# yoxu515/aot-benchmark

Hardware: NVIDIA H100
Metric: frames/sec (480p, 10 obj) (higher is better)
Workload: dtype f32

## Files before the change

### aot_benchmark_b200/csrc/conv_tc.cu

```cuda
#include <type_traits>

#include "common.cuh"
#include "tc_common.cuh"

namespace aotb {
namespace tc {

constexpr int CONV_A_BYTES = 128 * 128;

template <int BN>
__device__ __forceinline__ void wgmma_conv(float* acc, uint64_t a, uint64_t b) {
    if (BN == 256) wgmma_ss_n256(acc, a, b, 1u);
    else if (BN == 128) wgmma_ss_n128(acc, a, b, 1u);
    else wgmma_ss_n64(acc, a, b, 1u);
}

template <int BN>
__device__ __forceinline__ void conv_acc_to_staging(const float* acc, float* stg, int ld) {
    const int warp = threadIdx.x >> 5, lane = threadIdx.x & 31;
    const int row0 = (warp >> 2) * 64 + (warp & 3) * 16 + (lane >> 2), cq = (lane & 3) * 2;
#pragma unroll
    for (int j = 0; j < BN / 2; j += 2)
        *reinterpret_cast<float2*>(stg + (row0 + 8 * ((j >> 1) & 1)) * ld + 8 * (j >> 2) + cq) = make_float2(acc[j], acc[j + 1]);
}

struct ConvTcArgs {
    const float* in;
    const float* bias;
    const float* wscale;
    const float* res;
    float* out;
    int B, H, W, Cin, ldin;
    int Ho, Wo, Cout, ldout, ldres;
    int KH, KW, stride, pad;
    int M, nchunks;
    int act;
    int splits;
    int spin;
    long long* prof;
};

static int g_conv_tiling = 0;

struct RowInfo { int pix_base, iy0, ix0, valid; };

template <int BN, int S, int NB>
__device__ __forceinline__ void conv_finish_tile(const ConvTcArgs& a, const uint8_t* smem, int tid, int m0, int n0, int zrank) {
    constexpr int LD = BN + 4, C4 = BN / 4, RSTEP = 256 / C4, ROWS = 128 / S, ITERS = ROWS / RSTEP;
    constexpr int B = NB < ITERS ? NB : ITERS;
    static_assert(ITERS >= 1 && ITERS % B == 0, "finish tiling");
    const int c = (tid % C4) * 4, n = n0 + c;
    const int r0 = zrank * ROWS + tid / C4;
    const float4 b4 = a.bias ? __ldg(reinterpret_cast<const float4*>(a.bias + n)) : make_float4(0.f, 0.f, 0.f, 0.f);
    const float4 s4 = a.wscale ? __ldg(reinterpret_cast<const float4*>(a.wscale + n)) : make_float4(1.f, 1.f, 1.f, 1.f);
    const float* lbase = reinterpret_cast<const float*>(smem) + r0 * LD + c;
    const uint32_t sbase = smem_u32(lbase);
#pragma unroll 1
    for (int i0 = 0; i0 < ITERS; i0 += B) {
        float4 v[B][S], rs[B];
#pragma unroll
        for (int b = 0; b < B; ++b) {
            const int ro = (i0 + b) * RSTEP;
            if (S == 1) {
                v[b][0] = *reinterpret_cast<const float4*>(lbase + ro * LD);
            } else {
#pragma unroll
                for (int z = 0; z < S; ++z) v[b][z] = dsmem_ld_f4(dsmem_addr(sbase + (uint32_t)(ro * LD) * 4u, (uint32_t)z));
            }
            const int m = m0 + r0 + ro;
            rs[b] = (a.res && m < a.M) ? *reinterpret_cast<const float4*>(a.res + (size_t)m * a.ldres + n)
                                       : make_float4(0.f, 0.f, 0.f, 0.f);
        }
#pragma unroll
        for (int b = 0; b < B; ++b) {
            float4 o = v[b][0];
#pragma unroll
            for (int z = 1; z < S; ++z) { o.x += v[b][z].x; o.y += v[b][z].y; o.z += v[b][z].z; o.w += v[b][z].w; }
            o.x = fmaf(o.x, s4.x, b4.x); o.y = fmaf(o.y, s4.y, b4.y); o.z = fmaf(o.z, s4.z, b4.z); o.w = fmaf(o.w, s4.w, b4.w);
            o.x += rs[b].x; o.y += rs[b].y; o.z += rs[b].z; o.w += rs[b].w;
            o.x = apply_act(o.x, a.act); o.y = apply_act(o.y, a.act);
            o.z = apply_act(o.z, a.act); o.w = apply_act(o.w, a.act);
            const int m = m0 + r0 + (i0 + b) * RSTEP;
            if (m < a.M) *reinterpret_cast<float4*>(a.out + (size_t)m * a.ldout + n) = o;
        }
    }
}

template <int BN>
struct FinishPre { static constexpr int B = BN == 256 ? 4 : 8; float4 b4, s4; float4 rs[B]; };

template <int BN>
__device__ __forceinline__ void finish_prefetch(const ConvTcArgs& a, int tid, int m0, int n0, FinishPre<BN>& pre) {
    constexpr int C4 = BN / 4, RSTEP = 256 / C4;
    const int n = n0 + (tid % C4) * 4, r0 = tid / C4;
    pre.b4 = a.bias ? __ldg(reinterpret_cast<const float4*>(a.bias + n)) : make_float4(0.f, 0.f, 0.f, 0.f);
    pre.s4 = a.wscale ? __ldg(reinterpret_cast<const float4*>(a.wscale + n)) : make_float4(1.f, 1.f, 1.f, 1.f);
#pragma unroll
    for (int b = 0; b < FinishPre<BN>::B; ++b) {
        const int m = m0 + r0 + b * RSTEP;
        pre.rs[b] = (a.res && m < a.M) ? *reinterpret_cast<const float4*>(a.res + (size_t)m * a.ldres + n)
                                       : make_float4(0.f, 0.f, 0.f, 0.f);
    }
}

template <int BN>
__device__ __forceinline__ void conv_finish_tile_pre(const ConvTcArgs& a, const uint8_t* smem, int tid, int m0, int n0,
                                                     const FinishPre<BN>& pre) {
    constexpr int LD = BN + 4, C4 = BN / 4, RSTEP = 256 / C4, ITERS = 128 / RSTEP, B = FinishPre<BN>::B;
    static_assert(ITERS % B == 0, "finish tiling");
    const int c = (tid % C4) * 4, n = n0 + c, r0 = tid / C4;
    const uint32_t sbase = smem_u32(reinterpret_cast<const float*>(smem) + r0 * LD + c);
    float4 rs[B];
#pragma unroll
    for (int b = 0; b < B; ++b) rs[b] = pre.rs[b];
#pragma unroll 1
    for (int i0 = 0; i0 < ITERS; i0 += B) {
        float4 v[B], nx[B];
#pragma unroll
        for (int b = 0; b < B; ++b)
            asm volatile("ld.shared.v4.f32 {%0, %1, %2, %3}, [%4];" : "=f"(v[b].x), "=f"(v[b].y), "=f"(v[b].z), "=f"(v[b].w)
                         : "r"(sbase + (uint32_t)((i0 + b) * RSTEP * LD) * 4u));
        if (i0 + B < ITERS) {
#pragma unroll
            for (int b = 0; b < B; ++b) {
                const int m = m0 + r0 + (i0 + B + b) * RSTEP;
                nx[b] = (a.res && m < a.M) ? *reinterpret_cast<const float4*>(a.res + (size_t)m * a.ldres + n)
                                           : make_float4(0.f, 0.f, 0.f, 0.f);
            }
        }
#pragma unroll
        for (int b = 0; b < B; ++b) {
            float4 o = v[b];
            o.x = fmaf(o.x, pre.s4.x, pre.b4.x); o.y = fmaf(o.y, pre.s4.y, pre.b4.y);
            o.z = fmaf(o.z, pre.s4.z, pre.b4.z); o.w = fmaf(o.w, pre.s4.w, pre.b4.w);
            o.x += rs[b].x; o.y += rs[b].y; o.z += rs[b].z; o.w += rs[b].w;
            o.x = apply_act(o.x, a.act); o.y = apply_act(o.y, a.act);
            o.z = apply_act(o.z, a.act); o.w = apply_act(o.w, a.act);
            const int m = m0 + r0 + (i0 + b) * RSTEP;
            if (m < a.M) *reinterpret_cast<float4*>(a.out + (size_t)m * a.ldout + n) = o;
        }
        if (i0 + B < ITERS) {
#pragma unroll
            for (int b = 0; b < B; ++b) rs[b] = nx[b];
        }
    }
}

template <int BN, int STAGES, bool SPLIT>
struct ConvSmem {
    static constexpr int A_BYTES = CONV_A_BYTES;
    static constexpr int B_BYTES = BN * 128;
    static constexpr int PARTS = SPLIT ? 2 : 1;
    static constexpr int STAGE_BYTES = PARTS * A_BYTES + PARTS * B_BYTES;
    static constexpr int STG_LD = BN + 4;
    static_assert(128 * STG_LD * 4 <= STAGES * STAGE_BYTES, "staging tile must fit in the operand stages");
    static constexpr int TOTAL = STAGES * STAGE_BYTES + 128 * (int)sizeof(RowInfo) + 3 * STAGES * 8 + 1024;
    static_assert(TOTAL <= 227 * 1024, "shared memory of one CTA");
};

template <int BN, int STAGES, bool SPLIT>
__global__ void __launch_bounds__(384, 1)
conv_tc_kernel(const __grid_constant__ CUtensorMap tmWh, const __grid_constant__ CUtensorMap tmWl, const ConvTcArgs a) {
    using SM = ConvSmem<BN, STAGES, SPLIT>;
    extern __shared__ uint8_t smem_raw[];
    uint8_t* smem = reinterpret_cast<uint8_t*>((reinterpret_cast<uintptr_t>(smem_raw) + 1023) & ~(uintptr_t)1023);
    RowInfo* rinfo = reinterpret_cast<RowInfo*>(smem + STAGES * SM::STAGE_BYTES);
    uint64_t* a_full = reinterpret_cast<uint64_t*>(rinfo + 128);
    uint64_t* b_full = a_full + STAGES;
    uint64_t* s_free = b_full + STAGES;

    const int tid = threadIdx.x, warp = tid >> 5;
    const int m0 = blockIdx.x * 128, n0 = blockIdx.y * BN;
    long long* prof = a.prof ? a.prof + 12 * ((size_t)(blockIdx.z * gridDim.y + blockIdx.y) * gridDim.x + blockIdx.x) : nullptr;
    auto stamp = [&](int slot) { if (prof) prof[slot] = clock64(); };
    if (tid == 0) stamp(0);
    pdl_trigger();

    if (tid == 0) {
        for (int s = 0; s < STAGES; ++s) { mbar_init(&a_full[s], 128); mbar_init(&b_full[s], 1); mbar_init(&s_free[s], 8); }
        fence_mbar_init();
    }
    if (tid < 128) {
        const int m = m0 + tid;
        RowInfo ri;
        if (m < a.M) {
            const int HoWo = a.Ho * a.Wo;
            const int b = m / HoWo, r = m - b * HoWo;
            const int oy = r / a.Wo, ox = r - oy * a.Wo;
            ri.pix_base = b * a.H * a.W;
            ri.iy0 = oy * a.stride - a.pad;
            ri.ix0 = ox * a.stride - a.pad;
            ri.valid = 1;
        } else {
            ri.pix_base = 0; ri.iy0 = 0; ri.ix0 = 0; ri.valid = 0;
        }
        rinfo[tid] = ri;
    }
    __syncthreads();
    if (tid == 0) stamp(1);
    pdl_wait();
    const int cpt = (a.Cin % 64 == 0) ? (a.Cin >> 6) : 0;
    const int per = (a.nchunks + a.splits - 1) / a.splits;
    const int kbeg = blockIdx.z * per;
    const int nloc = max(0, min(per, a.nchunks - kbeg));

    FinishPre<BN> pre;
    const int wg = __shfl_sync(0xffffffffu, tid >> 7, 0);
    if (wg < 2) {
        const uint64_t dA0 = smem_desc_sw128(smem_u32(smem + wg * 64 * 128));
        const uint64_t dB0 = smem_desc_sw128(smem_u32(smem + SM::PARTS * SM::A_BYTES));
        float acc[BN / 2];
#pragma unroll
        for (int j = 0; j < BN / 2; ++j) acc[j] = 0.f;
#pragma unroll 1
        for (int it = 0; it < nloc; ++it) {
            const int s = it % STAGES;
            const uint32_t ph = (it / STAGES) & 1;
            mbar_wait_cp(&a_full[s], ph, a.spin);
            mbar_wait_cp(&b_full[s], ph, a.spin);
            if (it == 0 && tid == 0) stamp(3);
            const uint64_t so = (uint64_t)((s * SM::STAGE_BYTES) >> 4);
            const uint64_t ah = dA0 + so, al = ah + (SM::A_BYTES >> 4), bh = dB0 + so, bl = bh + (uint64_t)(SM::B_BYTES >> 4);
            reg_fence<BN / 2>(acc);
            wgmma_fence();
#pragma unroll
            for (int ks = 0; ks < 4; ++ks) {
                wgmma_conv<BN>(acc, ah + 2 * ks, bh + 2 * ks);
                if constexpr (SPLIT) {
                    wgmma_conv<BN>(acc, al + 2 * ks, bh + 2 * ks);
                    wgmma_conv<BN>(acc, ah + 2 * ks, bl + 2 * ks);
                }
            }
            wgmma_commit();
            reg_fence<BN / 2>(acc);
            wgmma_wait<1>();
            if (it > 0) mbar_arrive_warp(&s_free[(it - 1) % STAGES]);
        }
        wgmma_wait<0>();
        reg_fence<BN / 2>(acc);
        if (tid == 0) stamp(4);
        if (a.splits == 1) finish_prefetch<BN>(a, tid, m0, n0, pre);
        asm volatile("bar.sync 1, 256;" ::: "memory");
        conv_acc_to_staging<BN>(acc, reinterpret_cast<float*>(smem), SM::STG_LD);
        if (tid == 0) stamp(6);
    } else {
        const int p = tid - 256, q = p & 15, rsub = p >> 4;
        const uint32_t soff = rsub * 128 + (((q >> 1) ^ rsub) << 4) + ((q & 1) << 3);
        const float4* in4 = reinterpret_cast<const float4*>(a.in);
        uint32_t off[16];
        int cur_tap = -1, c4 = 0;
        if (p == 0) { tma_prefetch_desc(&tmWh); if constexpr (SPLIT) tma_prefetch_desc(&tmWl); }
        auto load_half = [&](int h, auto part_c, float4* v) {
            constexpr int part = decltype(part_c)::value;
            if (part == 0) {
                const int kc = kbeg + (h >> 1);
                int tap, c0;
                if (cpt > 0) { tap = kc / cpt; c0 = ((kc - tap * cpt) << 6) + q * 4; }
                else { const int k = kc * 64 + q * 4; tap = k / a.Cin; c0 = k - tap * a.Cin; }
                c4 = c0 >> 2;
                if (tap != cur_tap) {
                    cur_tap = tap;
                    const bool kvalid = tap < a.KH * a.KW;
                    const int ky = tap / a.KW, kx = tap - ky * a.KW;
#pragma unroll
                    for (int i = 0; i < 16; ++i) {
                        const RowInfo ri = rinfo[rsub + i * 8];
                        const int iy = ri.iy0 + ky, ix = ri.ix0 + kx;
                        off[i] = (kvalid && ri.valid && iy >= 0 && iy < a.H && ix >= 0 && ix < a.W)
                                     ? (uint32_t)(((size_t)(ri.pix_base + iy * a.W + ix) * a.ldin) >> 2)
                                     : ~0u;
                    }
                }
            }
#pragma unroll
            for (int i = 0; i < 8; ++i) {
                const uint32_t o = off[part * 8 + i];
                v[i] = o != ~0u ? __ldg(in4 + ((size_t)o + c4)) : make_float4(0.f, 0.f, 0.f, 0.f);
            }
        };
        auto store_half = [&](int h, auto part_c, const float4* v) {
            constexpr int part = decltype(part_c)::value;
            const int it = h >> 1, s = it % STAGES;
            uint8_t* stage = smem + s * SM::STAGE_BYTES;
            if (part == 0) {
                if (it >= STAGES) mbar_wait_cp(&s_free[s], ((it / STAGES) - 1) & 1, a.spin);
                if (p == 0) {
                    uint8_t* Bh = stage + SM::PARTS * SM::A_BYTES;
                    mbar_arrive_expect_tx(&b_full[s], SM::PARTS * SM::B_BYTES);
                    tma_load_2d(Bh, &tmWh, &b_full[s], (kbeg + it) * 64, n0);
                    if constexpr (SPLIT) tma_load_2d(Bh + SM::B_BYTES, &tmWl, &b_full[s], (kbeg + it) * 64, n0);
                }
            }
            uint8_t* Ah = stage + part * 64 * 128 + soff;
            uint8_t* Al = Ah + SM::A_BYTES;
#pragma unroll
            for (int i = 0; i < 8; ++i) {
                const __half2 h0 = __floats2half2_rn(v[i].x, v[i].y), h1 = __floats2half2_rn(v[i].z, v[i].w);
                if constexpr (!SPLIT) {
                    uint2 ph;
                    ph.x = *reinterpret_cast<const uint32_t*>(&h0); ph.y = *reinterpret_cast<const uint32_t*>(&h1);
                    *reinterpret_cast<uint2*>(Ah + i * 1024) = ph;
                    continue;
                }
                const __half2 l0 = __floats2half2_rn(v[i].x - __low2float(h0), v[i].y - __high2float(h0));
                const __half2 l1 = __floats2half2_rn(v[i].z - __low2float(h1), v[i].w - __high2float(h1));
                uint2 ph, pl;
                ph.x = *reinterpret_cast<const uint32_t*>(&h0); ph.y = *reinterpret_cast<const uint32_t*>(&h1);
                pl.x = *reinterpret_cast<const uint32_t*>(&l0); pl.y = *reinterpret_cast<const uint32_t*>(&l1);
                *reinterpret_cast<uint2*>(Ah + i * 1024) = ph;
                *reinterpret_cast<uint2*>(Al + i * 1024) = pl;
            }
            if (part == 1) {
                fence_proxy_async();
                mbar_arrive(&a_full[s]);
                if (it == 0 && p == 0) stamp(2);
            }
        };
        using P0 = std::integral_constant<int, 0>;
        using P1 = std::integral_constant<int, 1>;
        const int nh = 2 * nloc;
        float4 v0[8], v1[8], v2[8];
        if (nh > 0) { load_half(0, P0{}, v0); load_half(1, P1{}, v1); }
#pragma unroll 1
        for (int h = 0; h < nh; h += 6) {
            if (h + 2 < nh) load_half(h + 2, P0{}, v2);
            store_half(h, P0{}, v0);
            if (h + 3 < nh) load_half(h + 3, P1{}, v0);
            store_half(h + 1, P1{}, v1);
            if (h + 2 < nh) {
                if (h + 4 < nh) load_half(h + 4, P0{}, v1);
                store_half(h + 2, P0{}, v2);
                if (h + 5 < nh) load_half(h + 5, P1{}, v2);
                store_half(h + 3, P1{}, v0);
            }
            if (h + 4 < nh) {
                if (h + 6 < nh) load_half(h + 6, P0{}, v0);
                store_half(h + 4, P0{}, v1);
                if (h + 7 < nh) load_half(h + 7, P1{}, v1);
                store_half(h + 5, P1{}, v2);
            }
        }
        if (p == 0) stamp(5);
    }
    __syncwarp();
    if (a.splits > 1) cluster_sync_all(); else __syncthreads();
    if (tid == 0) stamp(8);
    if (warp < 8) {
        const int zr = a.splits > 1 ? (int)blockIdx.z : 0;
        if (a.splits == 1) conv_finish_tile_pre<BN>(a, smem, tid, m0, n0, pre);
        else if (a.splits == 2) conv_finish_tile<BN, 2, 4>(a, smem, tid, m0, n0, zr);
        else if (a.splits == 4) conv_finish_tile<BN, 4, 2>(a, smem, tid, m0, n0, zr);
        else conv_finish_tile<BN, 8, 2>(a, smem, tid, m0, n0, zr);
    }
    if (tid == 0) stamp(9);
    if (a.splits > 1) {
        __syncwarp();
        cluster_sync_all();
    }
    if (tid == 0) stamp(7);
}

static int make_tmap_weights(CUtensorMap* out, const void* base, int Kpad, int Cout, int BN) {
    PFN_encodeTiled fn = tensor_map_encoder();
    if (!fn) return AOTB_ERR_CUDA;
    cuuint64_t dims[2] = {(cuuint64_t)Kpad, (cuuint64_t)Cout};
    cuuint64_t strides[1] = {(cuuint64_t)Kpad * 2};
    cuuint32_t box[2] = {64, (cuuint32_t)BN};
    cuuint32_t estr[2] = {1, 1};
    CUresult r = fn(out, CU_TENSOR_MAP_DATA_TYPE_FLOAT16, 2, const_cast<void*>(base), dims, strides, box, estr,
                    CU_TENSOR_MAP_INTERLEAVE_NONE, CU_TENSOR_MAP_SWIZZLE_128B, CU_TENSOR_MAP_L2_PROMOTION_L2_256B,
                    CU_TENSOR_MAP_FLOAT_OOB_FILL_NONE);
    if (r != CUDA_SUCCESS) {
        set_error("cuTensorMapEncodeTiled(weights) failed (%d)", (int)r);
        return AOTB_ERR_CUDA;
    }
    return AOTB_OK;
}

template <int BN, int STAGES, bool SPLIT>
static int launch_conv_tc(const CUtensorMap& th, const CUtensorMap& tl, const ConvTcArgs& a, cudaStream_t st) {
    constexpr int smem = ConvSmem<BN, STAGES, SPLIT>::TOTAL;
    static bool configured = false;
    if (!configured) {
        cudaError_t e = cudaFuncSetAttribute(conv_tc_kernel<BN, STAGES, SPLIT>, cudaFuncAttributeMaxDynamicSharedMemorySize,
                                             smem);
        if (e != cudaSuccess) {
            set_error("aotb_conv2d_nhwc_tc: cudaFuncSetAttribute: %s", cudaGetErrorString(e));
            return AOTB_ERR_CUDA;
        }
        configured = true;
    }
    dim3 grid(cdiv(a.M, 128), a.Cout / BN, a.splits);
    launch_cluster(conv_tc_kernel<BN, STAGES, SPLIT>, dim3(grid), dim3(384), smem, st, a.splits, th, tl, a);
    return check_launch("aotb_conv2d_nhwc_tc");
}

}
}

using namespace aotb;

extern "C" int aotb_set_conv_tiling(int mode) {
    AOTB_REQUIRE(mode >= 0 && mode < (1 << 12), "aotb_set_conv_tiling: mode is a 12-bit mask");
    tc::g_conv_tiling = mode;
    return AOTB_OK;
}

extern "C" int aotb_conv2d_nhwc_tc(const float* in, const void* wh, const void* wl, const float* bias, const float* wscale,
                                   const float* res, float* out, int B, int H, int W, int Cin, int ldin, int Cout, int ldout, int ldres,
                                   int KH, int KW, int stride, int pad, int act, void* workspace, size_t workspace_bytes,
                                   void* stream) {
    AOTB_REQUIRE(in && wh && out, "aotb_conv2d_nhwc_tc: null pointer");
    const bool split = wl != nullptr;
    AOTB_REQUIRE(Cin % 4 == 0 && Cout % 64 == 0, "aotb_conv2d_nhwc_tc: Cin must be a multiple of 4, Cout of 64");
    AOTB_REQUIRE(act >= aotb::ACT_NONE && act <= aotb::ACT_RELU6, "aotb_conv2d_nhwc_tc: activation %d not supported (0-4)", act);
    AOTB_REQUIRE(ldin % 4 == 0 && ldout % 4 == 0 && (!res || ldres % 4 == 0) && ((uintptr_t)in % 16 == 0) &&
                     ((uintptr_t)out % 16 == 0) && (!res || (uintptr_t)res % 16 == 0) && (!bias || (uintptr_t)bias % 16 == 0) &&
                     (!wscale || (uintptr_t)wscale % 16 == 0),
                 "aotb_conv2d_nhwc_tc: 16-byte alignment required");
    AOTB_REQUIRE((size_t)B * H * W * ldin / 4 < 0xFFFFFFFFull, "aotb_conv2d_nhwc_tc: input larger than 2^32 float4");
    tc::ConvTcArgs a;
    a.in = in; a.bias = bias; a.wscale = wscale; a.res = res; a.out = out;
    a.B = B; a.H = H; a.W = W; a.Cin = Cin; a.ldin = ldin;
    a.Ho = (H + 2 * pad - KH) / stride + 1;
    a.Wo = (W + 2 * pad - KW) / stride + 1;
    AOTB_REQUIRE(a.Ho > 0 && a.Wo > 0, "aotb_conv2d_nhwc_tc: empty output");
    a.Cout = Cout; a.ldout = ldout; a.ldres = ldres; a.KH = KH; a.KW = KW; a.stride = stride; a.pad = pad;
    a.M = B * a.Ho * a.Wo;
    const int K = ((KH * KW * Cin + 63) / 64) * 64;
    a.nchunks = K / 64;
    a.act = act;
    const int mt = cdiv(a.M, 128);
    int BN = 64, best_s = 1;
    const float kGather = 2.5f, kGather1 = 2.0f;
    if ((tc::g_conv_tiling & 1) == 0) {
        float best = 1e30f;
        const int bns[3] = {256, 128, 64};
        const float t_chunk[3] = {fmaxf(kGather, 4.0f), fmaxf(kGather, 2.0f), fmaxf(kGather, 1.0f)};
        const float t_chunk1[3] = {fmaxf(kGather1, 4.0f / 3), fmaxf(kGather1, 2.0f / 3), fmaxf(kGather1, 1.0f / 3)};
        const float t_fin[3] = {8.0f, 4.0f, 2.0f};
        for (int bi = 0; bi < 3; ++bi) {
            if (Cout % bns[bi]) continue;
            for (int sp = 1; sp <= 8; sp <<= 1) {
                if (sp > a.nchunks) break;
                const int ctas = mt * (Cout / bns[bi]) * sp;
                const int slots = sp == 8 ? 128 : 132;
                if (sp > 1 && ctas > slots) continue;
                const int waves = cdiv(ctas, slots);
                const float t = waves * (3.0f + cdiv(a.nchunks, sp) * (split ? t_chunk[bi] : t_chunk1[bi]) + t_fin[bi]);
                if (t < best) { best = t; BN = bns[bi]; best_s = sp; }
            }
        }
    } else {
        if (Cout % 128 == 0 && mt * (Cout / 128) >= 120) BN = 128;
        const int ctas = mt * (Cout / BN);
        if (ctas < 100 && a.nchunks >= 4) {
            best_s = 8;
            while (best_s > 1 && (ctas * best_s > 160 || a.nchunks / best_s < 2)) best_s >>= 1;
        }
    }
    const int force_bn = (tc::g_conv_tiling >> 4) & 15, force_s = (tc::g_conv_tiling >> 8) & 15;
    if (force_bn) {
        BN = 32 << force_bn;
        AOTB_REQUIRE((BN == 64 || BN == 128 || BN == 256) && Cout % BN == 0, "aotb_conv2d_nhwc_tc: forced tile %d invalid", BN);
    }
    a.splits = force_bn ? 1 : best_s;
    const int ctas = mt * (Cout / BN);
    if (force_s) {
        AOTB_REQUIRE((force_s == 1 || force_s == 2 || force_s == 4 || force_s == 8) && force_s <= a.nchunks,
                     "aotb_conv2d_nhwc_tc: forced split %d invalid", force_s);
        a.splits = force_s;
    }
    a.spin = (tc::g_conv_tiling & 2) ? 1 : 0;
    a.prof = nullptr;
    if (tc::g_conv_tiling & 4) {
        const size_t need = (size_t)ctas * a.splits * 12 * sizeof(long long);
        AOTB_REQUIRE(workspace && workspace_bytes >= need, "aotb_conv2d_nhwc_tc: profile mode needs %zu workspace bytes", need);
        a.prof = (long long*)workspace;
    }
    CUtensorMap th, tl;
    int rc;
    if ((rc = tc::make_tmap_weights(&th, wh, K, Cout, BN)) != AOTB_OK) return rc;
    cudaStream_t st = (cudaStream_t)stream;
    if (!split) {
        if (BN == 256) return tc::launch_conv_tc<256, 4, false>(th, th, a, st);
        if (BN == 128) return tc::launch_conv_tc<128, 6, false>(th, th, a, st);
        return tc::launch_conv_tc<64, 8, false>(th, th, a, st);
    }
    if ((rc = tc::make_tmap_weights(&tl, wl, K, Cout, BN)) != AOTB_OK) return rc;
    if (BN == 256) return tc::launch_conv_tc<256, 2, true>(th, tl, a, st);
    if (BN == 128) return tc::launch_conv_tc<128, 3, true>(th, tl, a, st);
    return tc::launch_conv_tc<64, 4, true>(th, tl, a, st);
}
```

### aot_benchmark_b200/ops.py

```python
from __future__ import annotations

import contextlib
import os

import torch

from ._lib import AotbError, check, lib

ACT_NONE, ACT_RELU, ACT_GELU, ACT_SILU, ACT_RELU6, ACT_HSWISH = 0, 1, 2, 3, 4, 5
EW_COPY, EW_ADD, EW_MUL, EW_SILU, EW_SILU_MUL, EW_FILL = 0, 1, 2, 3, 4, 5


def _st(stream):
    return torch.cuda.current_stream().cuda_stream if stream is None else stream


def _chk(*ts):
    for t in ts:
        if t is None:
            continue
        if not t.is_cuda or t.dtype != torch.float32:
            raise AotbError(f"aot_benchmark_b200 kernels need float32 CUDA tensors, got {t.dtype} on {t.device}")
        if t.dim() >= 1 and t.stride(-1) != 1:
            raise AotbError("innermost stride must be 1")
# ... 67 lines not shown
        wt = torch.nn.functional.pad(wt, (0, 64 - K % 64))
    hi = wt.half()
    lo = (wt - hi.float()).half()
    return hi.contiguous(), lo.contiguous()


def weight_scale_exponents(w_kn):
    amax = w_kn.abs().amax(dim=0).float()
    _, ex = torch.frexp(amax)
    e = (14 - ex).clamp(max=126)
    return torch.where(amax > 0, e, torch.zeros_like(e)).to(torch.int32)


def split_fp16_scaled(w_kn):
    e = weight_scale_exponents(w_kn)
    hi, lo = split_fp16(w_kn.float() * _pow2(e))
    return hi, lo, _pow2(-e)


def _pow2(e):
    return ((e + 127) << 23).to(torch.int32).view(torch.float32)


CONV_CHAIN = False


def conv2d_tc(x, wh, wl, bias, out, res=None, KH=1, KW=1, stride=1, pad=0, act=ACT_NONE, stream=None, wscale=None):
    _chk(x, bias, out, res, wscale)
    B, H, W, Cin = x.shape
    Cout = wh.shape[0]
    ws = _tc_workspace(x.device)
    with _ConvProbe(2.0 * out.shape[0] * out.shape[1] * out.shape[2] * Cout * KH * KW * Cin, stream):
        check(lib().aotb_conv2d_nhwc_tc(_p(x), wh.data_ptr(), _p(wl), _p(bias), _p(wscale), _p(res), _p(out), B, H, W, Cin,
                                        _nhwc_ld(x), Cout, _nhwc_ld(out), _nhwc_ld(res) if res is not None else 0, KH, KW,
                                        stride, pad, act, ws.data_ptr(), ws.numel(), _st(stream)), "aotb_conv2d_nhwc_tc")
    return out


def conv2d(x, w, bias, out, res=None, KH=1, KW=1, stride=1, pad=0, dil=1, act=ACT_NONE, stream=None):
    if CONV_IMPL == "tc" and dil == 1:
        t = _TC_WEIGHTS.get(w.data_ptr())
        if t is not None:
            return conv2d_tc(x, t[0], None if _PRECISION == "fp16" else t[1], bias, out, res=res, KH=KH, KW=KW, stride=stride, pad=pad, act=act,
                             stream=stream, wscale=t[2])
    _chk(x, w, bias, out, res)
    B, H, W, Cin = x.shape
    Cout = w.shape[1]
    check(lib().aotb_conv2d_nhwc_f32(_p(x), _p(w), _p(bias), _p(res), _p(out), B, H, W, Cin, _nhwc_ld(x), Cout,
                                     _nhwc_ld(out), _nhwc_ld(res) if res is not None else 0, KH, KW, stride, pad,
                                     dil, act, _st(stream)), "aotb_conv2d_nhwc_f32")
    return out


def linear(x, wt, bias, out, res=None, act=ACT_NONE, stream=None):
    if CONV_IMPL == "tc":
        t = _TC_WEIGHTS.get(wt.data_ptr())
        if t is not None:
            _chk(x, bias, out, res, t[2])
            M, K = x.shape
            N = wt.shape[1]
            ws = _tc_workspace(x.device)
            with _ConvProbe(2.0 * M * N * K, stream):
                wl = None if _PRECISION == "fp16" else t[1]
                check(lib().aotb_conv2d_nhwc_tc(_p(x), t[0].data_ptr(), _p(wl), _p(bias), _p(t[2]), _p(res), _p(out),
                                                1, M, 1, K, x.stride(0), N, out.stride(0), res.stride(0) if res is not None else 0,
                                                1, 1, 1, 0, act, ws.data_ptr(), ws.numel(), _st(stream)),
                      "aotb_conv2d_nhwc_tc")
            return out
    _chk(x, wt, bias, out, res)
    M, K = x.shape
    N = wt.shape[1]
    check(lib().aotb_linear_f32(_p(x), _p(wt), _p(bias), _p(res), _p(out), M, K, x.stride(0), N, out.stride(0),
                                res.stride(0) if res is not None else 0, act, _st(stream)), "aotb_linear_f32")
    return out


def linear_tc(x, wh, wl, bias, out, res=None, act=ACT_NONE, stream=None):
    _chk(x, bias, out, res)
    if wh.dtype != torch.float16 or wl.dtype != torch.float16 or wh.shape != wl.shape or not wh.is_contiguous() \
            or not wl.is_contiguous():
        raise AotbError("linear_tc: wh / wl must be contiguous fp16 tensors of the same shape [N, K]")
    M, K = x.shape
    N = wh.shape[0]
    if wh.shape[1] != K or K % 64 or N % 64 or out.shape[0] != M or out.shape[1] != N:
        raise AotbError(f"linear_tc: shapes x {tuple(x.shape)}, w {tuple(wh.shape)}, out {tuple(out.shape)}")
    ws = _tc_workspace(x.device)
    check(lib().aotb_conv2d_nhwc_tc(_p(x), wh.data_ptr(), wl.data_ptr(), _p(bias), None, _p(res), _p(out), 1, M, 1, K,
                                    x.stride(0), N, out.stride(0), res.stride(0) if res is not None else 0, 1, 1, 1, 0,
                                    act, ws.data_ptr(), ws.numel(), _st(stream)), "aotb_conv2d_nhwc_tc")
# ... 534 lines not shown
```

### include/aotb200.h

```cpp
#ifndef AOTB200_H
#define AOTB200_H
#include <stddef.h>
#ifdef __cplusplus
extern "C" {
#endif

int aotb_version(void);
const char* aotb_arch(void);
const char* aotb_last_error_string(void);
unsigned long long aotb_launch_count(void);
void aotb_set_pdl(int on);
int aotb_set_conv_tiling(int mode);

int aotb_conv2d_nhwc_f32(const float* in, const float* w, const float* bias, const float* res, float* out,
                         int B, int H, int W, int Cin, int ldin, int Cout, int ldout, int ldres,
                         int KH, int KW, int stride, int pad, int dil, int act, void* stream);

int aotb_conv2d_nhwc_tc(const float* in, const void* wh, const void* wl, const float* bias, const float* wscale,
                        const float* res, float* out, int B, int H, int W, int Cin, int ldin, int Cout, int ldout, int ldres,
                        int KH, int KW, int stride, int pad, int act, void* workspace, size_t workspace_bytes,
                        void* stream);

int aotb_linear_f32(const float* in, const float* wt, const float* bias, const float* res, float* out,
                    int M, int K, int ldin, int N, int ldout, int ldres, int act, void* stream);

int aotb_nchw_to_nhwc_f32(const float* in, float* out, int B, int C, int HW, void* stream);
int aotb_nhwc_to_nchw_f32(const float* in, float* out, int B, int C, int HW, void* stream);
int aotb_image_to_nhwc4_f32(const float* in, float* out, int HW, void* stream);

int aotb_maxpool3x3s2_nhwc_f32(const float* in, float* out, int B, int H, int W, int C, void* stream);

int aotb_dwconv_nhwc_f32(const float* in, const float* w, const float* bias, float* out, int B, int H, int W,
                         int C, int ldin, int ldout, int KH, int KW, int stride, int pad, int dil, int act,
                         void* stream);

int aotb_bilinear_nhwc_f32(const float* in, float* out, int B, int H, int W, int C, int Ho, int Wo,
                           int align_corners, void* stream);

int aotb_eltwise_f32(int op, const float* a, int lda, const float* b, int ldb, float* out, int ldo,
                     int rows, int cols, float scalar, void* stream);
// ... 99 lines not shown
```

Before: 362.3.

## Make implicit-GEMM conv kernel persistent with fragment epilogue and pre-PDL weight prefetch

When split-K is off, the conv tensor-core kernel becomes persistent: each CTA loops over several output tiles, keeps the operand pipeline running across tiles, and double-buffers the row tables and bias/scale in shared memory. The epilogue now writes straight from wgmma accumulator fragments with L1 prefetch of the residual, instead of staging through shared memory. Weight TMA loads are issued before the PDL wait when the weights are flagged constant. The tiling cost model is updated for multi-tile CTAs. The risks are extra register pressure, uncoalesced float2 stores from the fragment epilogue, and more complex barrier logic.

```diff
diff --git a/aot_benchmark_b200/csrc/conv_tc.cu b/aot_benchmark_b200/csrc/conv_tc.cu
--- a/aot_benchmark_b200/csrc/conv_tc.cu
+++ b/aot_benchmark_b200/csrc/conv_tc.cu
@@ -33,14 +33,17 @@
     int B, H, W, Cin, ldin;
     int Ho, Wo, Cout, ldout, ldres;
     int KH, KW, stride, pad;
-    int M, nchunks;
+    int M, mtiles, nchunks;
     int act;
     int splits;
     int spin;
+    int const_w;
     long long* prof;
 };
 
+constexpr int AOTB_CONV_CONST_WEIGHTS = 256;
 static int g_conv_tiling = 0;
+static int g_conv_grid_cap = 0;
 
 struct RowInfo { int pix_base, iy0, ix0, valid; };
 
@@ -86,67 +89,65 @@
     }
 }
 
-template <int BN>
-struct FinishPre { static constexpr int B = BN == 256 ? 4 : 8; float4 b4, s4; float4 rs[B]; };
-
-template <int BN>
-__device__ __forceinline__ void finish_prefetch(const ConvTcArgs& a, int tid, int m0, int n0, FinishPre<BN>& pre) {
-    constexpr int C4 = BN / 4, RSTEP = 256 / C4;
-    const int n = n0 + (tid % C4) * 4, r0 = tid / C4;
-    pre.b4 = a.bias ? __ldg(reinterpret_cast<const float4*>(a.bias + n)) : make_float4(0.f, 0.f, 0.f, 0.f);
-    pre.s4 = a.wscale ? __ldg(reinterpret_cast<const float4*>(a.wscale + n)) : make_float4(1.f, 1.f, 1.f, 1.f);
-#pragma unroll
-    for (int b = 0; b < FinishPre<BN>::B; ++b) {
-        const int m = m0 + r0 + b * RSTEP;
-        pre.rs[b] = (a.res && m < a.M) ? *reinterpret_cast<const float4*>(a.res + (size_t)m * a.ldres + n)
-                                       : make_float4(0.f, 0.f, 0.f, 0.f);
-    }
-}
-
-template <int BN>
-__device__ __forceinline__ void conv_finish_tile_pre(const ConvTcArgs& a, const uint8_t* smem, int tid, int m0, int n0,
-                                                     const FinishPre<BN>& pre) {
-    constexpr int LD = BN + 4, C4 = BN / 4, RSTEP = 256 / C4, ITERS = 128 / RSTEP, B = FinishPre<BN>::B;
-    static_assert(ITERS % B == 0, "finish tiling");
-    const int c = (tid % C4) * 4, n = n0 + c, r0 = tid / C4;
-    const uint32_t sbase = smem_u32(reinterpret_cast<const float*>(smem) + r0 * LD + c);
-    float4 rs[B];
-#pragma unroll
-    for (int b = 0; b < B; ++b) rs[b] = pre.rs[b];
+__device__ __forceinline__ void prefetch_l1(const void* p) { asm volatile("prefetch.global.L1 [%0];" ::"l"(p)); }
+
+template <int BN, int ACT>
+__device__ __forceinline__ void conv_finish_frag(const ConvTcArgs& a, float* acc, const float* bs, int m0, int n0) {
+    constexpr bool ROLL = ACT == ACT_GELU || ACT == ACT_SILU;
+    constexpr int G = (ROLL || BN == 256) ? 1 : 8, NG = BN / 8, PF = 8;
+    const int warp = threadIdx.x >> 5, lane = threadIdx.x & 31;
+    const int r = m0 + (warp >> 2) * 64 + (warp & 3) * 16 + (lane >> 2);
+    const int c = (lane & 3) * 2;
+    const bool ok[2] = {r < a.M, r + 8 < a.M};
+    auto res_at = [&](int h, int k) { return a.res + (size_t)(r + 8 * h) * a.ldres + n0 + c + 8 * k; };
+    auto prefetch = [&](int k) {
+        if (G == 1 && a.res && k < NG) {
+            if (ok[0]) prefetch_l1(res_at(0, k));
+            if (ok[1]) prefetch_l1(res_at(1, k));
+        }
+    };
+    auto group = [&](int k, int h, float a0, float a1, float2 rs) {
+        const int n = c + 8 * k;
+        const float2 b2 = *reinterpret_cast<const float2*>(bs + n), s2 = *reinterpret_cast<const float2*>(bs + BN + n);
+        float ox = fmaf(a0, s2.x, b2.x), oy = fmaf(a1, s2.y, b2.y);
+        ox += rs.x; oy += rs.y;
+        ox = apply_act(ox, ACT); oy = apply_act(oy, ACT);
+        if (ok[h]) *reinterpret_cast<float2*>(a.out + (size_t)(r + 8 * h) * a.ldout + n0 + n) = make_float2(ox, oy);
+    };
+#pragma unroll
+    for (int k = 0; k < PF; ++k) prefetch(k);
+    if constexpr (ROLL) {
 #pragma unroll 1
-    for (int i0 = 0; i0 < ITERS; i0 += B) {
-        float4 v[B], nx[B];
-#pragma unroll
-        for (int b = 0; b < B; ++b)
-            asm volatile("ld.shared.v4.f32 {%0, %1, %2, %3}, [%4];" : "=f"(v[b].x), "=f"(v[b].y), "=f"(v[b].z), "=f"(v[b].w)
-                         : "r"(sbase + (uint32_t)((i0 + b) * RSTEP * LD) * 4u));
-        if (i0 + B < ITERS) {
-#pragma unroll
-            for (int b = 0; b < B; ++b) {
-                const int m = m0 + r0 + (i0 + B + b) * RSTEP;
-                nx[b] = (a.res && m < a.M) ? *reinterpret_cast<const float4*>(a.res + (size_t)m * a.ldres + n)
-                                           : make_float4(0.f, 0.f, 0.f, 0.f);
-            }
-        }
-#pragma unroll
-        for (int b = 0; b < B; ++b) {
-            float4 o = v[b];
-            o.x = fmaf(o.x, pre.s4.x, pre.b4.x); o.y = fmaf(o.y, pre.s4.y, pre.b4.y);
-            o.z = fmaf(o.z, pre.s4.z, pre.b4.z); o.w = fmaf(o.w, pre.s4.w, pre.b4.w);
-            o.x += rs[b].x; o.y += rs[b].y; o.z += rs[b].z; o.w += rs[b].w;
-            o.x = apply_act(o.x, a.act); o.y = apply_act(o.y, a.act);
-            o.z = apply_act(o.z, a.act); o.w = apply_act(o.w, a.act);
-            const int m = m0 + r0 + (i0 + b) * RSTEP;
-            if (m < a.M) *reinterpret_cast<float4*>(a.out + (size_t)m * a.ldout + n) = o;
-        }
-        if (i0 + B < ITERS) {
-#pragma unroll
-            for (int b = 0; b < B; ++b) rs[b] = nx[b];
-        }
-    }
-}
-
-template <int BN, int STAGES, bool SPLIT>
+        for (int k = 0; k < NG; ++k) {
+            prefetch(k + PF);
+            float2 rs[2];
+#pragma unroll
+            for (int h = 0; h < 2; ++h)
+                rs[h] = (a.res && ok[h]) ? *reinterpret_cast<const float2*>(res_at(h, k)) : make_float2(0.f, 0.f);
+#pragma unroll
+            for (int h = 0; h < 2; ++h) group(k, h, acc[2 * h], acc[2 * h + 1], rs[h]);
+#pragma unroll
+            for (int i = 0; i < BN / 2 - 4; ++i) acc[i] = acc[i + 4];
+        }
+    } else {
+#pragma unroll
+        for (int k0 = 0; k0 < NG; k0 += G) {
+            prefetch(k0 + PF);
+            float2 rs[G][2];
+#pragma unroll
+            for (int k = 0; k < G; ++k)
+#pragma unroll
+                for (int h = 0; h < 2; ++h)
+                    rs[k][h] = (a.res && ok[h]) ? *reinterpret_cast<const float2*>(res_at(h, k0 + k)) : make_float2(0.f, 0.f);
+#pragma unroll
+            for (int k = 0; k < G; ++k)
+#pragma unroll
+                for (int h = 0; h < 2; ++h) group(k0 + k, h, acc[4 * (k0 + k) + 2 * h], acc[4 * (k0 + k) + 2 * h + 1], rs[k][h]);
+        }
+    }
+}
+
+template <int BN, int STAGES, bool SPLIT, bool PERSIST>
 struct ConvSmem {
     static constexpr int A_BYTES = CONV_A_BYTES;
     static constexpr int B_BYTES = BN * 128;
@@ -154,34 +155,53 @@
     static constexpr int STAGE_BYTES = PARTS * A_BYTES + PARTS * B_BYTES;
     static constexpr int STG_LD = BN + 4;
     static_assert(128 * STG_LD * 4 <= STAGES * STAGE_BYTES, "staging tile must fit in the operand stages");
-    static constexpr int TOTAL = STAGES * STAGE_BYTES + 128 * (int)sizeof(RowInfo) + 3 * STAGES * 8 + 1024;
+    static constexpr int RTABLES = PERSIST ? 2 : 1, BS_FLOATS = PERSIST ? 2 * 2 * BN : 0;
+    static constexpr int TOTAL = STAGES * STAGE_BYTES + RTABLES * 128 * (int)sizeof(RowInfo) + BS_FLOATS * 4 + 3 * STAGES * 8 + 1024;
     static_assert(TOTAL <= 227 * 1024, "shared memory of one CTA");
 };
 
-template <int BN, int STAGES, bool SPLIT>
+template <int BN, int STAGES, bool SPLIT, bool PERSIST>
 __global__ void __launch_bounds__(384, 1)
 conv_tc_kernel(const __grid_constant__ CUtensorMap tmWh, const __grid_constant__ CUtensorMap tmWl, const ConvTcArgs a) {
-    using SM = ConvSmem<BN, STAGES, SPLIT>;
+    using SM = ConvSmem<BN, STAGES, SPLIT, PERSIST>;
     extern __shared__ uint8_t smem_raw[];
     uint8_t* smem = reinterpret_cast<uint8_t*>((reinterpret_cast<uintptr_t>(smem_raw) + 1023) & ~(uintptr_t)1023);
     RowInfo* rinfo = reinterpret_cast<RowInfo*>(smem + STAGES * SM::STAGE_BYTES);
-    uint64_t* a_full = reinterpret_cast<uint64_t*>(rinfo + 128);
+    float* bsm = reinterpret_cast<float*>(rinfo + SM::RTABLES * 128);
+    uint64_t* a_full = reinterpret_cast<uint64_t*>(bsm + SM::BS_FLOATS);
     uint64_t* b_full = a_full + STAGES;
     uint64_t* s_free = b_full + STAGES;
 
     const int tid = threadIdx.x, warp = tid >> 5;
-    const int m0 = blockIdx.x * 128, n0 = blockIdx.y * BN;
+    const int ntn = a.Cout / BN, ntiles = a.mtiles * ntn;
+    const int ntc = !PERSIST ? 1 : (int)blockIdx.x < ntiles ? (ntiles - 1 - (int)blockIdx.x) / (int)gridDim.x + 1 : 0;
+    auto tile_m0 = [&](int j) {
+        if constexpr (PERSIST) return ((int)(blockIdx.x + j * gridDim.x) / ntn) * 128;
+        else return (int)blockIdx.x * 128;
+    };
+    auto tile_n0 = [&](int j) {
+        if constexpr (PERSIST) return ((int)(blockIdx.x + j * gridDim.x) % ntn) * BN;
+        else return (int)blockIdx.y * BN;
+    };
     long long* prof = a.prof ? a.prof + 12 * ((size_t)(blockIdx.z * gridDim.y + blockIdx.y) * gridDim.x + blockIdx.x) : nullptr;
     auto stamp = [&](int slot) { if (prof) prof[slot] = clock64(); };
     if (tid == 0) stamp(0);
     pdl_trigger();
 
-    if (tid == 0) {
-        for (int s = 0; s < STAGES; ++s) { mbar_init(&a_full[s], 128); mbar_init(&b_full[s], 1); mbar_init(&s_free[s], 8); }
-        fence_mbar_init();
-    }
-    if (tid < 128) {
-        const int m = m0 + tid;
+    const int per = PERSIST ? a.nchunks : (a.nchunks + a.splits - 1) / a.splits;
+    const int kbeg = PERSIST ? 0 : blockIdx.z * per;
+    const int nloc = max(0, min(per, a.nchunks - kbeg));
+    const int nchk = ntc * nloc;
+    const int npre = a.const_w ? min(STAGES, nchk) : 0;
+    auto issue_b = [&](int g) {
+        const int j = PERSIST ? g / nloc : 0, it = g - j * nloc, s = g % STAGES;
+        uint8_t* Bh = smem + s * SM::STAGE_BYTES + SM::PARTS * SM::A_BYTES;
+        mbar_arrive_expect_tx(&b_full[s], SM::PARTS * SM::B_BYTES);
+        tma_load_2d(Bh, &tmWh, &b_full[s], (kbeg + it) * 64, tile_n0(j));
+        if constexpr (SPLIT) tma_load_2d(Bh + SM::B_BYTES, &tmWl, &b_full[s], (kbeg + it) * 64, tile_n0(j));
+    };
+    auto write_rows = [&](int j, int p) {
+        const int m = tile_m0(j) + p;
         RowInfo ri;
         if (m < a.M) {
             const int HoWo = a.Ho * a.Wo;
@@ -194,66 +214,107 @@
         } else {
             ri.pix_base = 0; ri.iy0 = 0; ri.ix0 = 0; ri.valid = 0;
         }
-        rinfo[tid] = ri;
+        rinfo[(j & 1) * 128 + p] = ri;
+    };
+
+    if (tid == 0) {
+        for (int s = 0; s < STAGES; ++s) { mbar_init(&a_full[s], 128); mbar_init(&b_full[s], 1); mbar_init(&s_free[s], 8); }
+        fence_mbar_init();
+    }
+    if (tid >= 256) {
+        for (int j = 0; j < min(ntc, 2); ++j) write_rows(j, tid - 256);
     }
     __syncthreads();
     if (tid == 0) stamp(1);
+    if (tid == 256) {
+        tma_prefetch_desc(&tmWh);
+        if constexpr (SPLIT) tma_prefetch_desc(&tmWl);
+        for (int g = 0; g < npre; ++g) issue_b(g);
+    }
     pdl_wait();
     const int cpt = (a.Cin % 64 == 0) ? (a.Cin >> 6) : 0;
-    const int per = (a.nchunks + a.splits - 1) / a.splits;
-    const int kbeg = blockIdx.z * per;
-    const int nloc = max(0, min(per, a.nchunks - kbeg));
-
-    FinishPre<BN> pre;
+
     const int wg = __shfl_sync(0xffffffffu, tid >> 7, 0);
     if (wg < 2) {
         const uint64_t dA0 = smem_desc_sw128(smem_u32(smem + wg * 64 * 128));
         const uint64_t dB0 = smem_desc_sw128(smem_u32(smem + SM::PARTS * SM::A_BYTES));
-        float acc[BN / 2];
-#pragma unroll
-        for (int j = 0; j < BN / 2; ++j) acc[j] = 0.f;
+        int g = 0;
 #pragma unroll 1
-        for (int it = 0; it < nloc; ++it) {
-            const int s = it % STAGES;
-            const uint32_t ph = (it / STAGES) & 1;
-            mbar_wait_cp(&a_full[s], ph, a.spin);
-            mbar_wait_cp(&b_full[s], ph, a.spin);
-            if (it == 0 && tid == 0) stamp(3);
-            const uint64_t so = (uint64_t)((s * SM::STAGE_BYTES) >> 4);
-            const uint64_t ah = dA0 + so, al = ah + (SM::A_BYTES >> 4), bh = dB0 + so, bl = bh + (uint64_t)(SM::B_BYTES >> 4);
+        for (int j = 0; j < ntc; ++j) {
+            float acc[BN / 2];
+#pragma unroll
+            for (int i = 0; i < BN / 2; ++i) acc[i] = 0.f;
+            float* bs = bsm + (j & 1) * 2 * BN;
+            if (PERSIST && tid < BN) {
+                const int n = tile_n0(j) + tid;
+                bs[tid] = a.bias ? __ldg(a.bias + n) : 0.f;
+                bs[BN + tid] = a.wscale ? __ldg(a.wscale + n) : 1.f;
+            }
+#pragma unroll 1
+            for (int it = 0; it < nloc; ++it, ++g) {
+                const int s = g % STAGES;
+                const uint32_t ph = (g / STAGES) & 1;
+                mbar_wait_cp(&a_full[s], ph, a.spin);
+                mbar_wait_cp(&b_full[s], ph, a.spin);
+                if (g == 0 && tid == 0) stamp(3);
+                const uint64_t so = (uint64_t)((s * SM::STAGE_BYTES) >> 4);
+                const uint64_t ah = dA0 + so, al = ah + (SM::A_BYTES >> 4), bh = dB0 + so, bl = bh + (uint64_t)(SM::B_BYTES >> 4);
+                reg_fence<BN / 2>(acc);
+                wgmma_fence();
+#pragma unroll
+                for (int ks = 0; ks < 4; ++ks) {
+                    wgmma_conv<BN>(acc, ah + 2 * ks, bh + 2 * ks);
+                    if constexpr (SPLIT) {
+                        wgmma_conv<BN>(acc, al + 2 * ks, bh + 2 * ks);
+                        wgmma_conv<BN>(acc, ah + 2 * ks, bl + 2 * ks);
+                    }
+                }
+                wgmma_commit();
+                reg_fence<BN / 2>(acc);
+                wgmma_wait<1>();
+                if (it > 0) mbar_arrive_warp(&s_free[(g - 1) % STAGES]);
+            }
+            wgmma_wait<0>();
             reg_fence<BN / 2>(acc);
-            wgmma_fence();
-#pragma unroll
-            for (int ks = 0; ks < 4; ++ks) {
-                wgmma_conv<BN>(acc, ah + 2 * ks, bh + 2 * ks);
-                if constexpr (SPLIT) {
-                    wgmma_conv<BN>(acc, al + 2 * ks, bh + 2 * ks);
-                    wgmma_conv<BN>(acc, ah + 2 * ks, bl + 2 * ks);
+            if (tid == 0) { if (PERSIST && j == 0) stamp(10); stamp(4); }
+            if constexpr (PERSIST) {
+                if (nloc > 0) mbar_arrive_warp(&s_free[(g - 1) % STAGES]);
+                asm volatile("bar.sync 1, 256;" ::: "memory");
+                const int m0 = tile_m0(j), n0 = tile_n0(j);
+                switch (a.act) {
+                    case ACT_RELU: conv_finish_frag<BN, ACT_RELU>(a, acc, bs, m0, n0); break;
+                    case ACT_GELU: conv_finish_frag<BN, ACT_GELU>(a, acc, bs, m0, n0); break;
+                    case ACT_SILU: conv_finish_frag<BN, ACT_SILU>(a, acc, bs, m0, n0); break;
+                    case ACT_RELU6: conv_finish_frag<BN, ACT_RELU6>(a, acc, bs, m0, n0); break;
+                    default: conv_finish_frag<BN, ACT_NONE>(a, acc, bs, m0, n0); break;
                 }
-            }
-            wgmma_commit();
-            reg_fence<BN / 2>(acc);
-            wgmma_wait<1>();
-            if (it > 0) mbar_arrive_warp(&s_free[(it - 1) % STAGES]);
-        }
-        wgmma_wait<0>();
-        reg_fence<BN / 2>(acc);
-        if (tid == 0) stamp(4);
-        if (a.splits == 1) finish_prefetch<BN>(a, tid, m0, n0, pre);
-        asm volatile("bar.sync 1, 256;" ::: "memory");
-        conv_acc_to_staging<BN>(acc, reinterpret_cast<float*>(smem), SM::STG_LD);
-        if (tid == 0) stamp(6);
+                if (tid == 0) { if (j == 0) stamp(8); stamp(9); }
+            } else {
+                asm volatile("bar.sync 1, 256;" ::: "memory");
+                conv_acc_to_staging<BN>(acc, reinterpret_cast<float*>(smem), SM::STG_LD);
+                if (tid == 0) stamp(6);
+            }
+        }
     } else {
         const int p = tid - 256, q = p & 15, rsub = p >> 4;
         const uint32_t soff = rsub * 128 + (((q >> 1) ^ rsub) << 4) + ((q & 1) << 3);
         const float4* in4 = reinterpret_cast<const float4*>(a.in);
         uint32_t off[16];
         int cur_tap = -1, c4 = 0;
-        if (p == 0) { tma_prefetch_desc(&tmWh); if constexpr (SPLIT) tma_prefetch_desc(&tmWl); }
+        const RowInfo* rows = rinfo;
         auto load_half = [&](int h, auto part_c, float4* v) {
             constexpr int part = decltype(part_c)::value;
             if (part == 0) {
-                const int kc = kbeg + (h >> 1);
+                const int g = h >> 1, j = PERSIST ? g / nloc : 0, it = g - j * nloc;
+                if (PERSIST && it == 0) {
+                    cur_tap = -1;
+                    rows = rinfo + (j & 1) * 128;
+                    if (j > 0) {
+                        asm volatile("bar.sync 2, 128;" ::: "memory");
+                        if (j + 1 < ntc) write_rows(j + 1, p);
+                    }
+                }
+                const int kc = kbeg + it;
                 int tap, c0;
                 if (cpt > 0) { tap = kc / cpt; c0 = ((kc - tap * cpt) << 6) + q * 4; }
                 else { const int k = kc * 64 + q * 4; tap = k / a.Cin; c0 = k - tap * a.Cin; }
@@ -264,7 +325,7 @@
                     const int ky = tap / a.KW, kx = tap - ky * a.KW;
 #pragma unroll
                     for (int i = 0; i < 16; ++i) {
-                        const RowInfo ri = rinfo[rsub + i * 8];
+                        const RowInfo ri = rows[rsub + i * 8];
                         const int iy = ri.iy0 + ky, ix = ri.ix0 + kx;
                         off[i] = (kvalid && ri.valid && iy >= 0 && iy < a.H && ix >= 0 && ix < a.W)
                                      ? (uint32_t)(((size_t)(ri.pix_base + iy * a.W + ix) * a.ldin) >> 2)
@@ -280,16 +341,11 @@
         };
         auto store_half = [&](int h, auto part_c, const float4* v) {
             constexpr int part = decltype(part_c)::value;
-            const int it = h >> 1, s = it % STAGES;
+            const int g = h >> 1, s = g % STAGES;
             uint8_t* stage = smem + s * SM::STAGE_BYTES;
             if (part == 0) {
-                if (it >= STAGES) mbar_wait_cp(&s_free[s], ((it / STAGES) - 1) & 1, a.spin);
-                if (p == 0) {
-                    uint8_t* Bh = stage + SM::PARTS * SM::A_BYTES;
-                    mbar_arrive_expect_tx(&b_full[s], SM::PARTS * SM::B_BYTES);
-                    tma_load_2d(Bh, &tmWh, &b_full[s], (kbeg + it) * 64, n0);
-                    if constexpr (SPLIT) tma_load_2d(Bh + SM::B_BYTES, &tmWl, &b_full[s], (kbeg + it) * 64, n0);
-                }
+                if (g >= STAGES) mbar_wait_cp(&s_free[s], ((g / STAGES) - 1) & 1, a.spin);
+                if (p == 0 && g >= npre) issue_b(g);
             }
             uint8_t* Ah = stage + part * 64 * 128 + soff;
             uint8_t* Al = Ah + SM::A_BYTES;
@@ -313,12 +369,12 @@
             if (part == 1) {
                 fence_proxy_async();
                 mbar_arrive(&a_full[s]);
-                if (it == 0 && p == 0) stamp(2);
+                if (g == 0 && p == 0) stamp(2);
             }
         };
         using P0 = std::integral_constant<int, 0>;
         using P1 = std::integral_constant<int, 1>;
-        const int nh = 2 * nloc;
+        const int nh = 2 * nchk;
         float4 v0[8], v1[8], v2[8];
         if (nh > 0) { load_half(0, P0{}, v0); load_half(1, P1{}, v1); }
 #pragma unroll 1
@@ -342,20 +398,21 @@
         }
         if (p == 0) stamp(5);
     }
-    __syncwarp();
-    if (a.splits > 1) cluster_sync_all(); else __syncthreads();
-    if (tid == 0) stamp(8);
-    if (warp < 8) {
-        const int zr = a.splits > 1 ? (int)blockIdx.z : 0;
-        if (a.splits == 1) conv_finish_tile_pre<BN>(a, smem, tid, m0, n0, pre);
-        else if (a.splits == 2) conv_finish_tile<BN, 2, 4>(a, smem, tid, m0, n0, zr);
-        else if (a.splits == 4) conv_finish_tile<BN, 4, 2>(a, smem, tid, m0, n0, zr);
-        else conv_finish_tile<BN, 8, 2>(a, smem, tid, m0, n0, zr);
-    }
-    if (tid == 0) stamp(9);
-    if (a.splits > 1) {
+    if constexpr (!PERSIST) {
         __syncwarp();
         cluster_sync_all();
+        if (tid == 0) stamp(8);
+        if (warp < 8) {
+            const int zr = (int)blockIdx.z, m0 = tile_m0(0), n0 = tile_n0(0);
+            if (a.splits == 2) conv_finish_tile<BN, 2, 4>(a, smem, tid, m0, n0, zr);
+            else if (a.splits == 4) conv_finish_tile<BN, 4, 2>(a, smem, tid, m0, n0, zr);
+            else conv_finish_tile<BN, 8, 2>(a, smem, tid, m0, n0, zr);
+        }
+        if (tid == 0) stamp(9);
+        __syncwarp();
+        cluster_sync_all();
+    } else if (tid == 0 && prof) {
+        prof[11] = ntc;
     }
     if (tid == 0) stamp(7);
 }
@@ -377,22 +434,43 @@
     return AOTB_OK;
 }
 
-template <int BN, int STAGES, bool SPLIT>
-static int launch_conv_tc(const CUtensorMap& th, const CUtensorMap& tl, const ConvTcArgs& a, cudaStream_t st) {
-    constexpr int smem = ConvSmem<BN, STAGES, SPLIT>::TOTAL;
+static int sm_count() {
+    static int n = 0;
+    if (n == 0) {
+        int dev = 0;
+        if (cudaGetDevice(&dev) != cudaSuccess || cudaDeviceGetAttribute(&n, cudaDevAttrMultiProcessorCount, dev) != cudaSuccess)
+            n = 132;
+    }
+    return n;
+}
+
+static dim3 conv_grid(const ConvTcArgs& a, int BN) {
+    if (a.splits > 1) return dim3(a.mtiles, a.Cout / BN, a.splits);
+    const int cap = g_conv_grid_cap > 0 ? g_conv_grid_cap : sm_count();
+    return dim3(min(a.mtiles * (a.Cout / BN), cap), 1, 1);
+}
+
+template <int BN, int STAGES, bool SPLIT, bool PERSIST>
+static int launch_conv_tc_as(const CUtensorMap& th, const CUtensorMap& tl, const ConvTcArgs& a, cudaStream_t st) {
+    constexpr int smem = ConvSmem<BN, STAGES, SPLIT, PERSIST>::TOTAL;
     static bool configured = false;
     if (!configured) {
-        cudaError_t e = cudaFuncSetAttribute(conv_tc_kernel<BN, STAGES, SPLIT>, cudaFuncAttributeMaxDynamicSharedMemorySize,
-                                             smem);
+        cudaError_t e = cudaFuncSetAttribute(conv_tc_kernel<BN, STAGES, SPLIT, PERSIST>,
+                                             cudaFuncAttributeMaxDynamicSharedMemorySize, smem);
         if (e != cudaSuccess) {
             set_error("aotb_conv2d_nhwc_tc: cudaFuncSetAttribute: %s", cudaGetErrorString(e));
             return AOTB_ERR_CUDA;
         }
         configured = true;
     }
-    dim3 grid(cdiv(a.M, 128), a.Cout / BN, a.splits);
-    launch_cluster(conv_tc_kernel<BN, STAGES, SPLIT>, dim3(grid), dim3(384), smem, st, a.splits, th, tl, a);
+    launch_cluster(conv_tc_kernel<BN, STAGES, SPLIT, PERSIST>, conv_grid(a, BN), dim3(384), smem, st, a.splits, th, tl, a);
     return check_launch("aotb_conv2d_nhwc_tc");
+}
+
+template <int BN, int STAGES, bool SPLIT>
+static int launch_conv_tc(const CUtensorMap& th, const CUtensorMap& tl, const ConvTcArgs& a, cudaStream_t st) {
+    return a.splits > 1 ? launch_conv_tc_as<BN, STAGES, SPLIT, false>(th, tl, a, st)
+                        : launch_conv_tc_as<BN, STAGES, SPLIT, true>(th, tl, a, st);
 }
 
 }
@@ -403,6 +481,12 @@
 extern "C" int aotb_set_conv_tiling(int mode) {
     AOTB_REQUIRE(mode >= 0 && mode < (1 << 12), "aotb_set_conv_tiling: mode is a 12-bit mask");
     tc::g_conv_tiling = mode;
+    return AOTB_OK;
+}
+
+extern "C" int aotb_set_conv_grid_cap(int ctas) {
+    AOTB_REQUIRE(ctas >= 0, "aotb_set_conv_grid_cap: negative cap");
+    tc::g_conv_grid_cap = ctas;
     return AOTB_OK;
 }
 
@@ -412,6 +496,8 @@
                                    void* stream) {
     AOTB_REQUIRE(in && wh && out, "aotb_conv2d_nhwc_tc: null pointer");
     const bool split = wl != nullptr;
+    const int const_w = (act & tc::AOTB_CONV_CONST_WEIGHTS) ? 1 : 0;
+    act &= ~tc::AOTB_CONV_CONST_WEIGHTS;
     AOTB_REQUIRE(Cin % 4 == 0 && Cout % 64 == 0, "aotb_conv2d_nhwc_tc: Cin must be a multiple of 4, Cout of 64");
     AOTB_REQUIRE(act >= aotb::ACT_NONE && act <= aotb::ACT_RELU6, "aotb_conv2d_nhwc_tc: activation %d not supported (0-4)", act);
     AOTB_REQUIRE(ldin % 4 == 0 && ldout % 4 == 0 && (!res || ldres % 4 == 0) && ((uintptr_t)in % 16 == 0) &&
@@ -427,27 +513,35 @@
     AOTB_REQUIRE(a.Ho > 0 && a.Wo > 0, "aotb_conv2d_nhwc_tc: empty output");
     a.Cout = Cout; a.ldout = ldout; a.ldres = ldres; a.KH = KH; a.KW = KW; a.stride = stride; a.pad = pad;
     a.M = B * a.Ho * a.Wo;
+    a.mtiles = cdiv(a.M, 128);
     const int K = ((KH * KW * Cin + 63) / 64) * 64;
     a.nchunks = K / 64;
     a.act = act;
+    a.const_w = const_w;
     const int mt = cdiv(a.M, 128);
     int BN = 64, best_s = 1;
     const float kGather = 2.5f, kGather1 = 2.0f;
     if ((tc::g_conv_tiling & 1) == 0) {
         float best = 1e30f;
         const int bns[3] = {256, 128, 64};
-        const float t_chunk[3] = {fmaxf(kGather, 4.0f), fmaxf(kGather, 2.0f), fmaxf(kGather, 1.0f)};
-        const float t_chunk1[3] = {fmaxf(kGather1, 4.0f / 3), fmaxf(kGather1, 2.0f / 3), fmaxf(kGather1, 1.0f / 3)};
+        const float t_mma[3] = {4.0f, 2.0f, 1.0f}, t_mma1[3] = {4.0f / 3, 2.0f / 3, 1.0f / 3};
         const float t_fin[3] = {8.0f, 4.0f, 2.0f};
         for (int bi = 0; bi < 3; ++bi) {
+            const float tf = t_fin[bi] * (bi == 0 && res ? 2.0f : 1.0f);
             if (Cout % bns[bi]) continue;
+            const float tm = split ? t_mma[bi] : t_mma1[bi], tc = fmaxf(split ? kGather : kGather1, tm);
             for (int sp = 1; sp <= 8; sp <<= 1) {
                 if (sp > a.nchunks) break;
                 const int ctas = mt * (Cout / bns[bi]) * sp;
                 const int slots = sp == 8 ? 128 : 132;
                 if (sp > 1 && ctas > slots) continue;
-                const int waves = cdiv(ctas, slots);
-                const float t = waves * (3.0f + cdiv(a.nchunks, sp) * (split ? t_chunk[bi] : t_chunk1[bi]) + t_fin[bi]);
+                float t;
+                if (sp == 1) {
+                    const int tpc = cdiv(ctas, 132);
+                    t = 3.0f + tpc * a.nchunks * tc + tf + (tpc - 1) * fmaxf(0.f, a.nchunks * (tm - tc) + tf);
+                } else {
+                    t = cdiv(ctas, slots) * (3.0f + cdiv(a.nchunks, sp) * tc + t_fin[bi]);
+                }
                 if (t < best) { best = t; BN = bns[bi]; best_s = sp; }
             }
         }
@@ -465,7 +559,6 @@
         AOTB_REQUIRE((BN == 64 || BN == 128 || BN == 256) && Cout % BN == 0, "aotb_conv2d_nhwc_tc: forced tile %d invalid", BN);
     }
     a.splits = force_bn ? 1 : best_s;
-    const int ctas = mt * (Cout / BN);
     if (force_s) {
         AOTB_REQUIRE((force_s == 1 || force_s == 2 || force_s == 4 || force_s == 8) && force_s <= a.nchunks,
                      "aotb_conv2d_nhwc_tc: forced split %d invalid", force_s);
@@ -474,7 +567,8 @@
     a.spin = (tc::g_conv_tiling & 2) ? 1 : 0;
     a.prof = nullptr;
     if (tc::g_conv_tiling & 4) {
-        const size_t need = (size_t)ctas * a.splits * 12 * sizeof(long long);
+        const dim3 grid = tc::conv_grid(a, BN);
+        const size_t need = (size_t)grid.x * grid.y * grid.z * 12 * sizeof(long long);
         AOTB_REQUIRE(workspace && workspace_bytes >= need, "aotb_conv2d_nhwc_tc: profile mode needs %zu workspace bytes", need);
         a.prof = (long long*)workspace;
     }
diff --git a/aot_benchmark_b200/ops.py b/aot_benchmark_b200/ops.py
--- a/aot_benchmark_b200/ops.py
+++ b/aot_benchmark_b200/ops.py
@@ -113,10 +113,13 @@
     return ((e + 127) << 23).to(torch.int32).view(torch.float32)
 
 
+CONV_CONST_WEIGHTS = 256
+
 CONV_CHAIN = False
 
 
-def conv2d_tc(x, wh, wl, bias, out, res=None, KH=1, KW=1, stride=1, pad=0, act=ACT_NONE, stream=None, wscale=None):
+def conv2d_tc(x, wh, wl, bias, out, res=None, KH=1, KW=1, stride=1, pad=0, act=ACT_NONE, stream=None, wscale=None,
+              const_w=False):
     _chk(x, bias, out, res, wscale)
     B, H, W, Cin = x.shape
     Cout = wh.shape[0]
@@ -124,7 +127,8 @@
     with _ConvProbe(2.0 * out.shape[0] * out.shape[1] * out.shape[2] * Cout * KH * KW * Cin, stream):
         check(lib().aotb_conv2d_nhwc_tc(_p(x), wh.data_ptr(), _p(wl), _p(bias), _p(wscale), _p(res), _p(out), B, H, W, Cin,
                                         _nhwc_ld(x), Cout, _nhwc_ld(out), _nhwc_ld(res) if res is not None else 0, KH, KW,
-                                        stride, pad, act, ws.data_ptr(), ws.numel(), _st(stream)), "aotb_conv2d_nhwc_tc")
+                                        stride, pad, act | (CONV_CONST_WEIGHTS if const_w else 0), ws.data_ptr(), ws.numel(),
+                                        _st(stream)), "aotb_conv2d_nhwc_tc")
     return out
 
 
@@ -133,7 +137,7 @@
         t = _TC_WEIGHTS.get(w.data_ptr())
         if t is not None:
             return conv2d_tc(x, t[0], None if _PRECISION == "fp16" else t[1], bias, out, res=res, KH=KH, KW=KW, stride=stride, pad=pad, act=act,
-                             stream=stream, wscale=t[2])
+                             stream=stream, wscale=t[2], const_w=True)
     _chk(x, w, bias, out, res)
     B, H, W, Cin = x.shape
     Cout = w.shape[1]
@@ -155,7 +159,7 @@
                 wl = None if _PRECISION == "fp16" else t[1]
                 check(lib().aotb_conv2d_nhwc_tc(_p(x), t[0].data_ptr(), _p(wl), _p(bias), _p(t[2]), _p(res), _p(out),
                                                 1, M, 1, K, x.stride(0), N, out.stride(0), res.stride(0) if res is not None else 0,
-                                                1, 1, 1, 0, act, ws.data_ptr(), ws.numel(), _st(stream)),
+                                                1, 1, 1, 0, act | CONV_CONST_WEIGHTS, ws.data_ptr(), ws.numel(), _st(stream)),
                       "aotb_conv2d_nhwc_tc")
             return out
     _chk(x, wt, bias, out, res)
diff --git a/include/aotb200.h b/include/aotb200.h
--- a/include/aotb200.h
+++ b/include/aotb200.h
@@ -11,11 +11,13 @@
 unsigned long long aotb_launch_count(void);
 void aotb_set_pdl(int on);
 int aotb_set_conv_tiling(int mode);
+int aotb_set_conv_grid_cap(int ctas);
 
 int aotb_conv2d_nhwc_f32(const float* in, const float* w, const float* bias, const float* res, float* out,
                          int B, int H, int W, int Cin, int ldin, int Cout, int ldout, int ldres,
                          int KH, int KW, int stride, int pad, int dil, int act, void* stream);
 
+#define AOTB_CONV_CONST_WEIGHTS 256
 int aotb_conv2d_nhwc_tc(const float* in, const void* wh, const void* wl, const float* bias, const float* wscale,
                         const float* res, float* out, int B, int H, int W, int Cin, int ldin, int Cout, int ldout, int ldres,
                         int KH, int KW, int stride, int pad, int act, void* workspace, size_t workspace_bytes,
```

New measurement: 388.6 (median of 6 runs). 7.3% higher.
